# XuanchenLi/Topo4D

Hardware: AMD Instinct MI355X
Metric: rasterizer fwd+bwd views/sec (higher is better)
Workload: dtype f32

## Files before the change

### topo4d_amd/csrc/t4d_raster_gaussian_bwd.h

```cpp
__device__ __forceinline__ void preprocess_bwd(const KP &kp)
{
    const uint32_t nblocks = (uint32_t)(kp.P + kBlock - 1) / kBlock;
    const uint32_t n_pv = gaussian_grid(kp.P, kp.V);
    const bool spare = blockIdx.x >= n_pv;
    uint32_t gb = 0, vb = 0;
    if (!spare && !block_and_view(blockIdx.x, (uint32_t)kp.V, nblocks, gb, vb)) return;
    const int v = spare ? (int)(blockIdx.x - n_pv) : (int)vb;
    const int g = (int)gb * kBlock + threadIdx.x;
    if (spare) {
        __shared__ float s_w[4];
        const float4 *td = reinterpret_cast<const float4 *>(kp.tile_dot) + (size_t)v * kp.T;
        const float *vb = kp.views + (size_t)v * T4D_VIEW_FLOATS + 35;
        const bool black = vb[0] == 0.f && vb[1] == 0.f && vb[2] == 0.f;
        const uint32_t *tc = kp.tile_count + (size_t)v * kp.T;
        float a = 0.f;
        for (int t = threadIdx.x; t < kp.T; t += kBlock) {
            if (tc[t] == 0u && black) continue;
            const float4 d4 = td[t];
            a += (d4.x + d4.y) + (d4.z + d4.w);
        }
        a = wave_sum_to_lane63(a);
        if ((threadIdx.x & 63) == 63) s_w[threadIdx.x >> 6] = a;
        __syncthreads();
        if (threadIdx.x == 0) kp.cotangent_dot[v] = kp.status->overflow != 0u ? 0.f : (s_w[0] + s_w[1]) + (s_w[2] + s_w[3]);
        return;
    }
    if (g >= kp.P) return;
    const size_t vg = (size_t)v * kp.P + g;
    const size_t gp = param_row0(kp, v) + (size_t)g;
    const ViewRecord vrec = load_view_record(kp.views, v);
    const float *view = vrec.view, *proj = vrec.proj;
    const uint32_t flag = kp.status->overflow;
    const int radius_in = kp.radii[vg];
    const float2 p2 = kp.xy[vg];
    const uint32_t base = kp.pair_off[vg];
    const float4 cq = kp.conic_opacity[vg];
    const float mean[3] = { kp.means3D[3 * gp], kp.means3D[3 * gp + 1], kp.means3D[3 * gp + 2] };
    float cov3_in[6] = { 0.f, 0.f, 0.f, 0.f, 0.f, 0.f };
    float4 q = make_float4(1.f, 0.f, 0.f, 0.f);
    float sc[3] = { 0.f, 0.f, 0.f };
    if (kp.cov3D_precomp) {
#pragma unroll
        for (int k = 0; k < 6; k++) cov3_in[k] = kp.cov3D_precomp[6 * gp + k];
    } else {
        sc[0] = kp.scales[3 * gp]; sc[1] = kp.scales[3 * gp + 1]; sc[2] = kp.scales[3 * gp + 2];
        q = reinterpret_cast<const float4 *>(kp.rotations)[gp];
    }
    const float4 q_raw = q;
    if (kp.raw_params && !kp.cov3D_precomp) {
        sc[0] = t4d_act_exp(sc[0]); sc[1] = t4d_act_exp(sc[1]); sc[2] = t4d_act_exp(sc[2]);
        q = t4d_act_normalize(q);
    }
    const bool truncated = flag != 0u;
    const int radius = truncated ? 0 : radius_in;

    float gm[3] = { 0.f, 0.f, 0.f }, g2x = 0.f, g2y = 0.f, gop = 0.f;
    float grgb[3] = { 0.f, 0.f, 0.f }, gsc[3] = { 0.f, 0.f, 0.f }, gq[4] = { 0.f, 0.f, 0.f, 0.f };
    float gcov[6] = { 0.f, 0.f, 0.f, 0.f, 0.f, 0.f };

    if (radius > 0) {
        int x0, y0, x1, y1;
        tile_rect(p2.x, p2.y, radius, kp.gx, kp.gy, x0, y0, x1, y1);
        const uint32_t npairs = (uint32_t)((x1 - x0) * (y1 - y0));
        const float2 *gp = reinterpret_cast<const float2 *>(kp.grad_pair) + (size_t)v * kp.cap * (kGP / 2);
        float S0 = 0.f, S1 = 0.f, S2 = 0.f, S3 = 0.f, S4 = 0.f, S5 = 0.f, gdep = 0.f;
        for (uint32_t k = 0; k < npairs; k++) {
            const uint32_t pr = base + k;
            if (pr >= kp.cap) break;
            const float2 *rec = gp + (size_t)pr * (kGP / 2);
            const float2 a0 = rec[0], a1 = rec[1], a2 = rec[2], a3 = rec[3], a4 = rec[4];
            S0 += a0.x; S1 += a0.y; S2 += a1.x; S3 += a1.y;
            S4 += a2.x; S5 += a2.y; grgb[0] += a3.x; grgb[1] += a3.y;
            grgb[2] += a4.x; gdep += a4.y;
        }
        gop = S0;
        g2x = -cq.w * (cq.x * S1 + cq.y * S2) * (0.5f * kp.W);
        g2y = -cq.w * (cq.z * S2 + cq.y * S1) * (0.5f * kp.H);
        const float X = -0.5f * cq.w * S3, Y = -cq.w * S4, Z = -0.5f * cq.w * S5;

        float cov3[6];
        if (kp.cov3D_precomp) {
#pragma unroll
            for (int k = 0; k < 6; k++) cov3[k] = cov3_in[k];
        } else {
            cov3d_from_scale_rot(sc, kp.scale_modifier, q, cov3);
        }
        const float tanx = vrec.tanx, tany = vrec.tany;
        const float fx = kp.W / (2.0f * tanx), fy = kp.H / (2.0f * tany);
        float T0[3], T1[3], t[3];
        bool inx, iny;
        ewa_rows(mean, view, fx, fy, tanx, tany, T0, T1, t, inx, iny);
        float v0[3], v1[3];
        sym3_mul(cov3, T0, v0);
        sym3_mul(cov3, T1, v1);
        const float a = T0[0] * v0[0] + T0[1] * v0[1] + T0[2] * v0[2] + T4D_COV2D_DILATION;
        const float b = T0[0] * v1[0] + T0[1] * v1[1] + T0[2] * v1[2];
        const float c = T1[0] * v1[0] + T1[1] * v1[1] + T1[2] * v1[2] + T4D_COV2D_DILATION;
        const float denom = a * c - b * b;
        const float d2inv = 1.f / ((denom * denom) + T4D_CONIC_BWD_EPS);
        float dL_da = 0.f, dL_db = 0.f, dL_dc = 0.f;
        if (d2inv != 0.f) {
            dL_da = d2inv * (-c * c * X + b * c * Y + (denom - a * c) * Z);
            dL_dc = d2inv * (-a * a * Z + a * b * Y + (denom - a * c) * X);
            dL_db = d2inv * (2.f * b * c * X - (denom + 2.f * b * b) * Y + 2.f * a * b * Z);
            gcov[0] = T0[0] * T0[0] * dL_da + T0[0] * T1[0] * dL_db + T1[0] * T1[0] * dL_dc;
            gcov[3] = T0[1] * T0[1] * dL_da + T0[1] * T1[1] * dL_db + T1[1] * T1[1] * dL_dc;
            gcov[5] = T0[2] * T0[2] * dL_da + T0[2] * T1[2] * dL_db + T1[2] * T1[2] * dL_dc;
            gcov[1] = 2.f * T0[0] * T0[1] * dL_da + (T0[0] * T1[1] + T0[1] * T1[0]) * dL_db + 2.f * T1[0] * T1[1] * dL_dc;
            gcov[2] = 2.f * T0[0] * T0[2] * dL_da + (T0[0] * T1[2] + T0[2] * T1[0]) * dL_db + 2.f * T1[0] * T1[2] * dL_dc;
            gcov[4] = 2.f * T0[2] * T0[1] * dL_da + (T0[1] * T1[2] + T0[2] * T1[1]) * dL_db + 2.f * T1[1] * T1[2] * dL_dc;
        }
        float dJ00 = 0.f, dJ02 = 0.f, dJ11 = 0.f, dJ12 = 0.f;
#pragma unroll
        for (int j = 0; j < 3; j++) {
            const float dT0 = 2.f * v0[j] * dL_da + v1[j] * dL_db;
            const float dT1 = 2.f * v1[j] * dL_dc + v0[j] * dL_db;
            dJ00 += view[j * 4 + 0] * dT0; dJ02 += view[j * 4 + 2] * dT0;
            dJ11 += view[j * 4 + 1] * dT1; dJ12 += view[j * 4 + 2] * dT1;
        }
        const float tz = 1.f / t[2], tz2 = tz * tz, tz3 = tz2 * tz;
        const float dtx = (inx ? 1.f : 0.f) * -fx * tz2 * dJ02;
        const float dty = (iny ? 1.f : 0.f) * -fy * tz2 * dJ12;
        const float dtz = -fx * tz2 * dJ00 - fy * tz2 * dJ11 + (2.f * fx * t[0]) * tz3 * dJ02 + (2.f * fy * t[1]) * tz3 * dJ12;
        gm[0] = view[0] * dtx + view[1] * dty + view[2] * dtz;
        gm[1] = view[4] * dtx + view[5] * dty + view[6] * dtz;
        gm[2] = view[8] * dtx + view[9] * dty + view[10] * dtz;

        const float hx = proj[0] * mean[0] + proj[4] * mean[1] + proj[8] * mean[2] + proj[12];
        const float hy = proj[1] * mean[0] + proj[5] * mean[1] + proj[9] * mean[2] + proj[13];
        const float hw = proj[3] * mean[0] + proj[7] * mean[1] + proj[11] * mean[2] + proj[15];
        const float mw = 1.0f / (hw + T4D_HOM_W_EPS);
        const float mul1 = hx * mw * mw, mul2 = hy * mw * mw;
        gm[0] += (proj[0] * mw - proj[3] * mul1) * g2x + (proj[1] * mw - proj[3] * mul2) * g2y;
        gm[1] += (proj[4] * mw - proj[7] * mul1) * g2x + (proj[5] * mw - proj[7] * mul2) * g2y;
        gm[2] += (proj[8] * mw - proj[11] * mul1) * g2x + (proj[9] * mw - proj[11] * mul2) * g2y;
        gm[0] += view[2] * gdep; gm[1] += view[6] * gdep; gm[2] += view[10] * gdep;

        if (!kp.cov3D_precomp) {
            float R[9];
            quat_rot(q, R);
            const float s[3] = { kp.scale_modifier * sc[0], kp.scale_modifier * sc[1], kp.scale_modifier * sc[2] };
            const float Gs[9] = { gcov[0], 0.5f * gcov[1], 0.5f * gcov[2], 0.5f * gcov[1], gcov[3], 0.5f * gcov[4],
                                  0.5f * gcov[2], 0.5f * gcov[4], gcov[5] };
            float Mp[9], D[9];
#pragma unroll
            for (int r = 0; r < 3; r++)
#pragma unroll
                for (int k = 0; k < 3; k++) Mp[r * 3 + k] = R[r * 3 + k] * s[k];
#pragma unroll
            for (int k = 0; k < 3; k++) {
                float dM[3];
#pragma unroll
                for (int r = 0; r < 3; r++)
                    dM[r] = 2.f * (Gs[r * 3] * Mp[k] + Gs[r * 3 + 1] * Mp[3 + k] + Gs[r * 3 + 2] * Mp[6 + k]);
                gsc[k] = kp.scale_modifier * (dM[0] * R[k] + dM[1] * R[3 + k] + dM[2] * R[6 + k]);
#pragma unroll
                for (int r = 0; r < 3; r++) D[r * 3 + k] = dM[r] * s[k];
            }
            const float r = q.x, x = q.y, y = q.z, z = q.w;
            gq[0] = 2.f * z * (D[3] - D[1]) + 2.f * y * (D[2] - D[6]) + 2.f * x * (D[7] - D[5]);
            gq[1] = 2.f * y * (D[1] + D[3]) + 2.f * z * (D[2] + D[6]) + 2.f * r * (D[7] - D[5]) - 4.f * x * (D[4] + D[8]);
            gq[2] = 2.f * x * (D[1] + D[3]) + 2.f * r * (D[2] - D[6]) + 2.f * z * (D[5] + D[7]) - 4.f * y * (D[0] + D[8]);
            gq[3] = 2.f * r * (D[3] - D[1]) + 2.f * x * (D[2] + D[6]) + 2.f * y * (D[5] + D[7]) - 4.f * z * (D[0] + D[4]);
        }
    }

    if (kp.raw_params && radius > 0) {
        gop = t4d_act_sigmoid_bwd(cq.w, gop);
        if (!kp.cov3D_precomp) {
#pragma unroll
            for (int k = 0; k < 3; k++) gsc[k] = t4d_act_exp_bwd(sc[k], gsc[k]);
            const float4 gr = t4d_act_normalize_bwd(q_raw, make_float4(gq[0], gq[1], gq[2], gq[3]));
            gq[0] = gr.x; gq[1] = gr.y; gq[2] = gr.z; gq[3] = gr.w;
        }
    }
    kp.dL_dmeans3D[vg * 3] = gm[0]; kp.dL_dmeans3D[vg * 3 + 1] = gm[1]; kp.dL_dmeans3D[vg * 3 + 2] = gm[2];
    kp.dL_dmeans2D[vg * 3] = g2x; kp.dL_dmeans2D[vg * 3 + 1] = g2y; kp.dL_dmeans2D[vg * 3 + 2] = 0.f;
    kp.dL_dopacities[vg] = gop;
    if (kp.dL_dcolors) { kp.dL_dcolors[vg * 3] = grgb[0]; kp.dL_dcolors[vg * 3 + 1] = grgb[1]; kp.dL_dcolors[vg * 3 + 2] = grgb[2]; }
    if (kp.cov3D_precomp) {
#pragma unroll
        for (int k = 0; k < 6; k++) kp.dL_dcov3D[vg * 6 + k] = gcov[k];
    } else {
        kp.dL_dscales[vg * 3] = gsc[0]; kp.dL_dscales[vg * 3 + 1] = gsc[1]; kp.dL_dscales[vg * 3 + 2] = gsc[2];
        reinterpret_cast<float4 *>(kp.dL_drotations)[vg] = make_float4(gq[0], gq[1], gq[2], gq[3]);
    }
}

#ifndef T4D_PBWD_WAVES
#define T4D_PBWD_WAVES 7
#endif
__global__ __launch_bounds__(kBlock) __attribute__((amdgpu_waves_per_eu(T4D_PBWD_WAVES, T4D_PBWD_WAVES))) void k_preprocess_bwd(const KP kp)
{
    preprocess_bwd(kp);
}

__global__ __launch_bounds__(kBlock) void k_sh_bwd(const KP kp)
{
    __shared__ float s_bas[kBlock][17];
    __shared__ float s_gc[kBlock][4];
    const int tid = threadIdx.x;
    const uint32_t nblocks = (uint32_t)(kp.P + kBlock - 1) / kBlock;
    uint32_t pblock, vb;
    if (!block_and_view(blockIdx.x, (uint32_t)kp.V, nblocks, pblock, vb)) return;
    const int v = (int)vb;
    const int g0 = (int)pblock * kBlock;
    const int n = min(kBlock, kp.P - g0);
    const int M3 = kp.M * 3;
    if (tid < n) {
        const int g = g0 + tid;
        const size_t vg = (size_t)v * kp.P + g;
        const size_t gp = param_row0(kp, v) + (size_t)g;
        const bool vis = kp.status->overflow == 0u && kp.radii[vg] > 0;
        float gc[3] = { 0.f, 0.f, 0.f };
        float bas[16];
#pragma unroll
        for (int i = 0; i < 16; i++) bas[i] = 0.f;
        if (vis) {
            const float *vr = kp.views + (size_t)v * T4D_VIEW_FLOATS;
            const float d0[3] = { kp.means3D[3 * gp] - vr[32], kp.means3D[3 * gp + 1] - vr[33], kp.means3D[3 * gp + 2] - vr[34] };
            const float len = sqrtf(d0[0] * d0[0] + d0[1] * d0[1] + d0[2] * d0[2]);
            const float d[3] = { d0[0] / len, d0[1] / len, d0[2] / len };
            float bx[16], by[16], bz[16];
            sh_basis(kp.deg, d, bas);
            sh_basis_grad(kp.deg, d, bx, by, bz);
            const uint32_t cl = kp.clamped[vg];
            const float *grgb = kp.dL_dcolors + vg * 3;
            gc[0] = (cl & 1u) ? 0.f : grgb[0]; gc[1] = (cl & 2u) ? 0.f : grgb[1]; gc[2] = (cl & 4u) ? 0.f : grgb[2];
            const int K = (kp.deg + 1) * (kp.deg + 1);
            float gd[3] = { 0.f, 0.f, 0.f };
            const float *sh = kp.shs + gp * M3;
            if ((kp.M & 3) == 0 && K == 16) {
                const float4 *sh4 = reinterpret_cast<const float4 *>(sh);
                float c[48];
#pragma unroll
                for (int i = 0; i < 12; i++) { const float4 t4 = sh4[i]; c[4 * i] = t4.x; c[4 * i + 1] = t4.y; c[4 * i + 2] = t4.z; c[4 * i + 3] = t4.w; }
#pragma unroll
                for (int k = 0; k < 16; k++) {
                    const float t = c[3 * k] * gc[0] + c[3 * k + 1] * gc[1] + c[3 * k + 2] * gc[2];
                    gd[0] += bx[k] * t; gd[1] += by[k] * t; gd[2] += bz[k] * t;
                }
            } else {
#pragma unroll
                for (int k = 0; k < 16; k++) {
                    if (k < K) {
                        const float t = sh[k * 3] * gc[0] + sh[k * 3 + 1] * gc[1] + sh[k * 3 + 2] * gc[2];
                        gd[0] += bx[k] * t; gd[1] += by[k] * t; gd[2] += bz[k] * t;
                    } else {
                        bas[k] = 0.f;
                    }
                }
            }
            const float dot = d[0] * gd[0] + d[1] * gd[1] + d[2] * gd[2];
            float *gm = kp.dL_dmeans3D + vg * 3;
#pragma unroll
            for (int jj = 0; jj < 3; jj++) gm[jj] += (gd[jj] - d[jj] * dot) / len;
        }
#pragma unroll
        for (int i = 0; i < 16; i++) s_bas[tid][i] = bas[i];
        s_gc[tid][0] = gc[0]; s_gc[tid][1] = gc[1]; s_gc[tid][2] = gc[2];
    }
    __syncthreads();
    float *out = kp.dL_dshs + ((size_t)v * kp.P + g0) * M3;
    if (kp.M == 16) {
        float4 *out4 = reinterpret_cast<float4 *>(out);
        for (int i = tid; i < n * 12; i += kBlock) {
            const int slot = i / 12, e0 = (i % 12) * 4;
            float o[4];
#pragma unroll
            for (int e = 0; e < 4; e++) o[e] = s_bas[slot][(e0 + e) / 3] * s_gc[slot][(e0 + e) % 3];
            out4[i] = make_float4(o[0], o[1], o[2], o[3]);
        }
    } else {
        for (int i = tid; i < n * M3; i += kBlock) {
            const int slot = i / M3, e = i % M3, k = e / 3;
            out[i] = k < 16 ? s_bas[slot][k] * s_gc[slot][e % 3] : 0.f;
        }
    }
}

#ifndef T4D_SHB_VIEWS
#define T4D_SHB_VIEWS 8
#endif
__global__ __launch_bounds__(kBlock) void k_sh_bwd16(const KP kp)
{
    constexpr int kPitch = 52;
    __shared__ __attribute__((aligned(16))) float s_raw[kBlock * kPitch];
    float (*s_bas)[17] = reinterpret_cast<float (*)[17]>(s_raw);
    float (*s_gc)[4] = reinterpret_cast<float (*)[4]>(s_raw + kBlock * 17);
    static_assert(kBlock * 17 + kBlock * 4 <= kBlock * kPitch && (kBlock * 17) % 4 == 0, "the exchange arrays live inside the staging area");
    const int tid = threadIdx.x;
    const uint32_t nblocks = (uint32_t)(kp.P + kBlock - 1) / kBlock;
    const uint32_t ngroups = (uint32_t)(kp.V + T4D_SHB_VIEWS - 1) / T4D_SHB_VIEWS;
    uint32_t pblock, vgrp;
    if (!block_and_view(blockIdx.x, ngroups, nblocks, pblock, vgrp)) return;
    const int g0 = (int)pblock * kBlock;
    const int n = min(kBlock, kp.P - g0);
    const size_t row0 = param_row0(kp, (int)vgrp * T4D_SHB_VIEWS);
    {
        const float4 *src = reinterpret_cast<const float4 *>(kp.shs + (row0 + (size_t)g0) * 48);
        for (int i = tid; i < n * 12; i += kBlock) {
            const int r = i / 12, part = i - r * 12;
            *reinterpret_cast<float4 *>(s_raw + r * kPitch + part * 4) = src[i];
        }
    }
    __syncthreads();
    float c[48];
#pragma unroll
    for (int i = 0; i < 12; i++) {
        const float4 t4 = *reinterpret_cast<const float4 *>(s_raw + min(tid, n - 1) * kPitch + 4 * i);
        c[4 * i] = t4.x; c[4 * i + 1] = t4.y; c[4 * i + 2] = t4.z; c[4 * i + 3] = t4.w;
    }
    __syncthreads();
    const int g = g0 + min(tid, n - 1);
    const float mean[3] = { kp.means3D[3 * (row0 + (size_t)g)], kp.means3D[3 * (row0 + (size_t)g) + 1], kp.means3D[3 * (row0 + (size_t)g) + 2] };
    const bool truncated = kp.status->overflow != 0u;
    const int v_end = min(kp.V, (int)(vgrp + 1u) * T4D_SHB_VIEWS);
    for (int v = (int)vgrp * T4D_SHB_VIEWS; v < v_end; v++) {
        if (tid < n) {
            const size_t vg = (size_t)v * kp.P + g;
            const bool vis = !truncated && kp.radii[vg] > 0;
            float gc[3] = { 0.f, 0.f, 0.f };
            float bas[16];
#pragma unroll
            for (int i = 0; i < 16; i++) bas[i] = 0.f;
            if (vis) {
                const float *vr = kp.views + (size_t)v * T4D_VIEW_FLOATS;
                const float d0[3] = { mean[0] - vr[32], mean[1] - vr[33], mean[2] - vr[34] };
                const float len = sqrtf(d0[0] * d0[0] + d0[1] * d0[1] + d0[2] * d0[2]);
                const float d[3] = { d0[0] / len, d0[1] / len, d0[2] / len };
                float bx[16], by[16], bz[16];
                sh_basis(3, d, bas);
                sh_basis_grad(3, d, bx, by, bz);
                const uint32_t cl = kp.clamped[vg];
                const float *grgb = kp.dL_dcolors + vg * 3;
                gc[0] = (cl & 1u) ? 0.f : grgb[0]; gc[1] = (cl & 2u) ? 0.f : grgb[1]; gc[2] = (cl & 4u) ? 0.f : grgb[2];
                float gd[3] = { 0.f, 0.f, 0.f };
#pragma unroll
                for (int k = 0; k < 16; k++) {
                    const float t = c[3 * k] * gc[0] + c[3 * k + 1] * gc[1] + c[3 * k + 2] * gc[2];
                    gd[0] += bx[k] * t; gd[1] += by[k] * t; gd[2] += bz[k] * t;
                }
                const float dot = d[0] * gd[0] + d[1] * gd[1] + d[2] * gd[2];
                float *gm = kp.dL_dmeans3D + vg * 3;
#pragma unroll
                for (int jj = 0; jj < 3; jj++) gm[jj] += (gd[jj] - d[jj] * dot) / len;
            }
#pragma unroll
            for (int i = 0; i < 16; i++) s_bas[tid][i] = bas[i];
            s_gc[tid][0] = gc[0]; s_gc[tid][1] = gc[1]; s_gc[tid][2] = gc[2];
        }
        __syncthreads();
        float4 *out4 = reinterpret_cast<float4 *>(kp.dL_dshs + ((size_t)v * kp.P + g0) * 48);
        for (int i = tid; i < n * 12; i += kBlock) {
            const int slot = i / 12, e0 = (i - slot * 12) * 4;
            float o[4];
#pragma unroll
            for (int e = 0; e < 4; e++) o[e] = s_bas[slot][(e0 + e) / 3] * s_gc[slot][(e0 + e) % 3];
            out4[i] = make_float4(o[0], o[1], o[2], o[3]);
        }
        __syncthreads();
    }
}

constexpr int kDotBlocks = 64;

__global__ __launch_bounds__(kBlock) void k_view_dot_partial(const float *a, const float *b, size_t n, float *partial)
{
    __shared__ float s_w[4];
    const int v = blockIdx.y, blk = blockIdx.x, tid = threadIdx.x;
    const float *pa = a + (size_t)v * n, *pb = b + (size_t)v * n;
    const size_t per = (((n + kDotBlocks - 1) / kDotBlocks) + 3) & ~(size_t)3;
    const size_t lo = min(n, (size_t)blk * per), hi = min(n, lo + per);
    float acc = 0.f;
    if ((n & 3) == 0 && (((uintptr_t)a | (uintptr_t)b) & 15) == 0) {
        for (size_t i = lo + (size_t)tid * 4; i < hi; i += (size_t)kBlock * 4) {
            const float4 x = *reinterpret_cast<const float4 *>(pa + i), y = *reinterpret_cast<const float4 *>(pb + i);
            acc += (x.x * y.x + x.y * y.y) + (x.z * y.z + x.w * y.w);
        }
    } else {
        for (size_t k = lo + tid; k < hi; k += kBlock) acc += pa[k] * pb[k];
    }
    acc = wave_sum_to_lane63(acc);
    if ((tid & 63) == 63) s_w[tid >> 6] = acc;
    __syncthreads();
    if (tid == 0) partial[(size_t)v * kDotBlocks + blk] = (s_w[0] + s_w[1]) + (s_w[2] + s_w[3]);
}

__global__ __launch_bounds__(64) void k_view_dot_final(const float *partial, float *out)
{
    const int v = blockIdx.x;
    float x = partial[(size_t)v * kDotBlocks + threadIdx.x];
    x = wave_sum_to_lane63(x);
    if (threadIdx.x == 63) out[v] = x;
}

__global__ __launch_bounds__(kBlock) void k_mark_visible(int P, const float *means3D, const float *view, uint8_t *present)
{
#pragma clang fp contract(off)
    const int g = blockIdx.x * kBlock + threadIdx.x;
    if (g >= P) return;
    const float z = view[2] * means3D[3 * (size_t)g] + view[6] * means3D[3 * (size_t)g + 1] +
                    view[10] * means3D[3 * (size_t)g + 2] + view[14];
    present[g] = z > T4D_NEAR_CULL_Z ? 1 : 0;
}
```

### topo4d_amd/csrc/t4d_raster_render_bwd.h

```cpp
__device__ __forceinline__ void tile_pixel_bwd(int tid, int tx, int ty, int &px, int &py)
{
    const int w = tid >> 6, r = (tid >> 4) & 3, i = tid & 15;
    px = tx * T4D_TILE_X + ((w & 1) << 3) + ((r & 1) << 2) + (i >> 2);
    py = ty * T4D_TILE_Y + ((w >> 1) << 3) + ((r >> 1) << 2) + (i & 3);
}

__device__ __forceinline__ int fwd_thread_of(int tid) { return (tid & ~15) | ((tid & 3) << 2) | ((tid >> 2) & 3); }

struct RowWeights { float X, ks, kg; };

__device__ __forceinline__ RowWeights row_weights(const int lane)
{
    const int r = lane >> 4, i = lane & 15, bank = i >> 2, b1 = (i >> 1) & 1;
    RowWeights k;
    k.X = (float)(((r & 1) << 2) + (i >> 2)) - 3.5f;
    const float y0 = (float)((r >> 1) << 2) - 3.5f;
    const float Y = y0 + (float)(i & 3), Yp = y0 + (float)((i & 3) ^ 2);
    auto Ka = [&](float y) { return bank == 1 ? y * y : (bank == 3 ? 0.f : 1.f); };
    auto Kb = [&](float y) { return (bank & 1) ? 0.f : y; };
    k.ks = b1 ? Kb(Y) : Ka(Y);
    k.kg = b1 ? Kb(Yp) : Ka(Yp);
    return k;
}

template <bool NINE>
__device__ __forceinline__ float reduce_moments_row(const float e, const float ex, const float exx, const float c0, const float c1,
                                                    const float c2, const float cd, const RowWeights &k)
{
    float a, b, c;
#define T4D_RED_X                                                                                     \
        "s_nop 1\n\t"                                                                                 \
        "v_add_f32_dpp %[a], %[v0], %[v0] row_ror:8 row_mask:0xf bank_mask:0xf\n\t"                   \
        "v_add_f32_dpp %[b], %[v2], %[v2] row_ror:8 row_mask:0xf bank_mask:0xf\n\t"                   \
        "v_add_f32_dpp %[c], %[v4], %[v4] row_ror:8 row_mask:0xf bank_mask:0xf\n\t"                   \
        "v_add_f32_dpp %[a], %[v1], %[v1] row_ror:8 row_mask:0xf bank_mask:0xc\n\t"                   \
        "v_add_f32_dpp %[b], %[v3], %[v3] row_ror:8 row_mask:0xf bank_mask:0xc\n\t"                   \
        "v_add_f32_dpp %[c], %[v5], %[v5] row_ror:8 row_mask:0xf bank_mask:0xc\n\t"
#define T4D_RED_X4                                                                                    \
        "v_add_f32_dpp %[a], %[a], %[a] row_shl:4 row_mask:0xf bank_mask:0x5\n\t"                     \
        "v_add_f32_dpp %[a], %[b], %[b] row_shr:4 row_mask:0xf bank_mask:0xa\n\t"                     \
        "v_add_f32_dpp %[b], %[c], %[c] row_shl:4 row_mask:0xf bank_mask:0x5\n\t"                     \
        "v_add_f32_dpp %[b], %[c], %[c] row_shr:4 row_mask:0xf bank_mask:0xa\n\t"
#define T4D_RED_OUT [a] "=&v"(a), [b] "=&v"(b), [c] "=&v"(c)
#define T4D_RED_IN [v0] "v"(exx), [v1] "v"(c0), [v2] "v"(c1), [v3] "v"(c2), [v4] "v"(e), [v5] "v"(ex), [ks] "v"(k.ks), [kg] "v"(k.kg), \
                   [m0] "s"(0xaaaaaaaaaaaaaaaaull)
    if (NINE) {
        asm(T4D_RED_X T4D_RED_X4
            "v_add_f32_dpp %[a], %[a], %[a] quad_perm:[2,3,0,1] row_mask:0xf bank_mask:0xf\n\t"
            "v_mul_f32_e32 %[c], %[b], %[ks]\n\t"
            "v_fmac_f32_dpp %[c], %[b], %[kg] quad_perm:[2,3,0,1] row_mask:0xf bank_mask:0xf\n\t"
            "v_cndmask_b32_e64 %[b], %[a], %[c], %[m0]\n\t"
            "v_cndmask_b32_e64 %[c], %[c], %[a], %[m0]\n\t"
            "s_nop 0\n\t"
            "v_add_f32_dpp %[c], %[b], %[c] quad_perm:[1,0,3,2] row_mask:0xf bank_mask:0xf"
            : T4D_RED_OUT : T4D_RED_IN);
        return c;
    } else {
        float d;
        asm(T4D_RED_X
            "v_add_f32_dpp %[d], %[v6], %[v6] row_ror:8 row_mask:0xf bank_mask:0xf\n\t"
            T4D_RED_X4
            "v_add_f32_dpp %[d], %[d], %[d] row_ror:4 row_mask:0xf bank_mask:0xf\n\t"
            "v_cndmask_b32_e64 %[c], %[d], %[a], %[m1]\n\t"
            "v_cndmask_b32_e64 %[d], %[a], %[d], %[m1]\n\t"
            "v_mul_f32_e32 %[a], %[b], %[ks]\n\t"
            "v_fmac_f32_dpp %[a], %[b], %[kg] quad_perm:[2,3,0,1] row_mask:0xf bank_mask:0xf\n\t"
            "v_add_f32_dpp %[d], %[c], %[d] quad_perm:[2,3,0,1] row_mask:0xf bank_mask:0xf\n\t"
            "v_cndmask_b32_e64 %[b], %[d], %[a], %[m0]\n\t"
            "v_cndmask_b32_e64 %[a], %[a], %[d], %[m0]\n\t"
            "s_nop 0\n\t"
            "v_add_f32_dpp %[a], %[b], %[a] quad_perm:[1,0,3,2] row_mask:0xf bank_mask:0xf"
            : T4D_RED_OUT, [d] "=&v"(d) : T4D_RED_IN, [v6] "v"(cd), [m1] "s"(0xccccccccccccccccull));
        return a;
    }
#undef T4D_RED_X
#undef T4D_RED_X4
#undef T4D_RED_OUT
#undef T4D_RED_IN
}

__device__ __forceinline__ int row10_index(const int lane)
{
    const int b0 = lane & 1, b1 = (lane >> 1) & 1, bank = (lane >> 2) & 3;
    if (!b0) {
        if (bank == 0) return b1 ? 2 : 0;
        if (bank == 1) return b1 ? -1 : 5;
        if (bank == 2) return b1 ? 4 : 1;
        return -1;
    }
    if (!b1) return bank == 0 ? 3 : (bank == 1 ? 7 : (bank == 2 ? 6 : 8));
    return bank == 0 ? 9 : -1;
}

__device__ __forceinline__ void moments_about_centre(float (&m)[10], const float pxf, const float pyf)
{
    const double px = pxf, py = pyf, M00 = m[0], M10 = m[1], M01 = m[2], M20 = m[3], M11 = m[4], M02 = m[5];
    const double sx = fma(px, M00, -M10), sy = fma(py, M00, -M01);
    m[1] = (float)sx; m[2] = (float)sy;
    m[3] = (float)fma(px, sx, -fma(px, M10, -M20));
    m[4] = (float)fma(px, sy, -fma(py, M10, -M11));
    m[5] = (float)fma(py, sy, -fma(py, M01, -M02));
}

__device__ __forceinline__ float moment_e(const float e) { return __uint_as_float(__float_as_uint(e) & 0xffffffc0u); }

__device__ __forceinline__ uint32_t row_max_u32(uint32_t v)
{
    v = max(v, (uint32_t)__builtin_amdgcn_update_dpp(0, (int)v, 0xB1, 0xf, 0xf, true));
    v = max(v, (uint32_t)__builtin_amdgcn_update_dpp(0, (int)v, 0x4E, 0xf, 0xf, true));
    v = max(v, (uint32_t)__builtin_amdgcn_update_dpp(0, (int)v, 0x141, 0xf, 0xf, true));
    v = max(v, (uint32_t)__builtin_amdgcn_update_dpp(0, (int)v, 0x140, 0xf, 0xf, true));
    return v;
}

#ifndef T4D_BWD_WAVES
#define T4D_BWD_WAVES 5
#endif
#ifndef T4D_SEG_WAVES
#define T4D_SEG_WAVES 5
#endif
#ifndef T4D_BWD_DA_WAVES
#define T4D_BWD_DA_WAVES T4D_BWD_WAVES
#endif
#define T4D_BWD_NW (LAT ? 2 : (SEGN != 0 ? T4D_SEG_WAVES : (DA ? T4D_BWD_DA_WAVES : T4D_BWD_WAVES)))
#define T4D_BWD_ATTR __attribute__((amdgpu_waves_per_eu(LAT ? 1 : T4D_BWD_NW, T4D_BWD_NW)))
constexpr int kAcc = 10;
constexpr int kEmptySpan = 64;
template <bool DA, bool LAT, int SEGN, bool LONG = false>
__global__ __launch_bounds__(kBlock) T4D_BWD_ATTR void k_render_bwd(const KP kp)
{
    constexpr bool SEG = SEGN != 0;
    constexpr int kSeg = SEG ? SEGN : ::kSeg;
    constexpr int kBwdBatch = SEG ? SEGN : ::kBwdBatch;
    constexpr int kSlabs = LAT ? 16 : 4;
    constexpr int kChunks = (kBwdBatch + 63) / 64;
    constexpr int kListStride = kBwdBatch + 4;
    constexpr int kEnt = 40;
    static_assert(kBwdBatch % 64 == 0, "staged slots come in chunks of one per lane");
    static_assert(kGP == kAcc, "the slab entry and the scratch record hold the same ten sums");
    static_assert(kAcc * 4 == kEnt, "a slab entry and a staged record must have the same stride");
    struct __attribute__((aligned(16))) Shared {
        unsigned char rec[(kBwdBatch + 1) * kEnt];
        float acc[kSlabs][kBwdBatch + 1][kAcc];
        unsigned short list[4][4][kListStride];
        float cut_r2[kChunks * 64];
        uint32_t pair[kBwdBatch];
        uint32_t wmax[4];
    };
    static_assert(((kBwdBatch + 1) * kEnt) % 8 == 0 && (sizeof(float) * kSlabs * (kBwdBatch + 1) * kAcc) % 8 == 0 &&
                  (sizeof(unsigned short) * 16 * kListStride) % 8 == 0, "8-byte members must stay 8-byte aligned");
    __shared__ Shared sh;
    auto &s_rec = sh.rec;
    auto &s_pair = sh.pair;
    auto &s_acc = sh.acc;
    auto &s_r2 = sh.cut_r2;
    auto &s_wmax = sh.wmax;
    auto &s_list = sh.list;
    constexpr int kNull = kBwdBatch;

    const int tid = threadIdx.x;
    const int wave = __builtin_amdgcn_readfirstlane(tid >> 6), lane = tid & 63, row = lane >> 4;
    const int my_slot = (!DA && row10_index(lane & 15) == 9) ? -1 : row10_index(lane & 15);
    const RowWeights rw = row_weights(lane);
    if (tid == 0) {
#pragma unroll
        for (int k = 0; k < kEnt / 8; k++) reinterpret_cast<float2 *>(s_rec + kNull * kEnt)[k] = make_float2(0.f, 0.f);
    }
    if (blockIdx.x >= kp.tile_blocks) {
        const uint32_t spans = (uint32_t)(kp.T + kEmptySpan - 1) / kEmptySpan;
        const uint32_t j = blockIdx.x - kp.tile_blocks;
        const int v = (int)(j / spans), t0 = (int)(j % spans) * kEmptySpan;
        const float *vb = kp.views + (size_t)v * T4D_VIEW_FLOATS + 35;
        const float b0 = vb[0], b1 = vb[1], b2 = vb[2];
        if (b0 == 0.f && b1 == 0.f && b2 == 0.f) return;
        const size_t HWe = (size_t)kp.H * kp.W;
        const float *dc = kp.dL_dcolor + (size_t)v * 3 * HWe;
        for (int t = t0; t < min(t0 + kEmptySpan, kp.T); t++) {
            if (kp.tile_count[(size_t)v * kp.T + t] != 0u) continue;
            const int ty = t / kp.gx, tx = t - ty * kp.gx;
            int ex, ey;
            tile_pixel(tid, tx, ty, ex, ey);
            float d = 0.f;
            if (ex < kp.W && ey < kp.H) {
                const size_t pe = (size_t)ey * kp.W + ex;
                d = fmaf(b0, dc[pe], fmaf(b1, dc[HWe + pe], b2 * dc[2 * HWe + pe]));
            }
            d = wave_sum_to_lane63(d);
            if (lane == 63) kp.tile_dot[((size_t)v * kp.T + t) * 4 + wave] = d;
        }
        return;
    }
    uint4 it;
    if (SEG && !LONG) {
        it = kp.slot_tab[blockIdx.x];
        if (it.w == 0u) return;
    }
    for (int i = tid; i < kSlabs * (kBwdBatch + 1) * kAcc; i += kBlock) (&s_acc[0][0][0])[i] = 0.f;
    for (uint32_t item = blockIdx.x; item < (SEG ? (LONG ? kp.status->live_segments : blockIdx.x + 1u) : (uint32_t)(kp.V * kp.T)); item += kp.tile_blocks) {
    if (SEG && LONG) it = kp.slot_tab[kp.live[item]];
    if (!SEG) it = kp.items[item];
    const int seg_j = SEG ? (int)(it.w & 0x7fffffffu) : 0;
    const int v = (int)(it.x >> 20), t_ = (int)(it.x & 0xfffffu);
    const int ty = t_ / kp.gx, tx = t_ - ty * kp.gx;
    const uint32_t off = it.y, n = it.z;
    if (n == 0) break;
    if (!SEG && LONG && n >= kp.seg_min_pairs &&
        kp.slot_tab[(size_t)v * kp.slots_per_view + seg_slot0(kp, off, (uint32_t)t_)].w != 0u) continue;
    const unsigned long long *keys = kp.keys + (size_t)v * kp.cap + off;
    const float *r2_in = kp.cut_r2 + (size_t)v * kp.cap + off;
    const float2 *xy = kp.xy + (size_t)v * kp.P;
    const float4 *co = kp.conic_opacity + (size_t)v * kp.P;
    const float *rgb = kp.shs ? kp.rgb + (size_t)v * kp.P * 3 : kp.colors_precomp + 3 * param_row0(kp, v);
    const int32_t *radii = kp.radii + (size_t)v * kp.P;
    const uint32_t *pair_off = kp.pair_off + (size_t)v * kp.P;
    float2 *grad_pair = reinterpret_cast<float2 *>(kp.grad_pair) + (size_t)v * kp.cap * (kGP / 2);
    const float *vr = kp.views + (size_t)v * T4D_VIEW_FLOATS;

    int px, py;
    tile_pixel_bwd(tid, tx, ty, px, py);
    const bool inside = px < kp.W && py < kp.H;
    const v2f pix_f = { (float)px, (float)py };
    const size_t HW = (size_t)kp.H * kp.W, pix = (size_t)py * kp.W + px;

    float T_final = 0.f, dp0 = 0.f, dp1 = 0.f, dp2 = 0.f, ddep = 0.f, dalp = 0.f;
    uint32_t last_contributor = 0;
    if (inside) {
        T_final = kp.final_T[(size_t)v * HW + pix];
        last_contributor = kp.n_contrib[(size_t)v * HW + pix];
        const float *dc = kp.dL_dcolor + (size_t)v * 3 * HW;
        dp0 = dc[pix]; dp1 = dc[HW + pix]; dp2 = dc[2 * HW + pix];
        if (DA && kp.dL_ddepth) ddep = kp.dL_ddepth[(size_t)v * HW + pix];
        if (DA && kp.dL_dalpha) dalp = kp.dL_dalpha[(size_t)v * HW + pix];
    }
    const v2f dp01 = { dp0, dp1 };
    float T = T_final;
    float acc = vr[35] * dp0 + vr[36] * dp1 + vr[37] * dp2;
    const int nb = (int)((n + kBwdBatch - 1) / kBwdBatch);
    if (SEG && seg_j + 1 < nb) {
        const uint32_t p = (uint32_t)(seg_j + 1) * kSeg;
        if (last_contributor > p) {
            const float *sb = kp.snap + ((size_t)v * kp.slots_per_view + seg_slot0(kp, off, (uint32_t)t_)) * (kSnapFloats * kBlock) + fwd_thread_of(tid);
            const float *sp = sb + (size_t)seg_j * (kSnapFloats * kBlock), *sf = sb + (size_t)(nb - 1) * (kSnapFloats * kBlock);
            const float Tp = sp[0];
            float suf = fmaf(sf[kBlock] - sp[kBlock], dp0, fmaf(sf[2 * kBlock] - sp[2 * kBlock], dp1, (sf[3 * kBlock] - sp[3 * kBlock]) * dp2));
            if (DA) suf = fmaf(sf[4 * kBlock] - sp[4 * kBlock], ddep, suf) + (Tp - T_final) * dalp;
            acc = fmaf(T_final, acc, suf) / Tp;
            T = Tp;
        }
    }

    const uint32_t rmax_v = row_max_u32(last_contributor);
    uint32_t row_max[4];
#pragma unroll
    for (int r = 0; r < 4; r++) row_max[r] = lane_value(rmax_v, 16 * r);
    const uint32_t wave_max = max(max(row_max[0], row_max[1]), max(row_max[2], row_max[3]));
    if (lane == 0) s_wmax[wave] = wave_max;
    __syncthreads();
    const uint32_t tile_max = max(max(s_wmax[0], s_wmax[1]), max(s_wmax[2], s_wmax[3]));

    for (int bi = SEG ? seg_j : nb - 1; bi >= (SEG ? seg_j : 0); bi--) {
        const uint32_t lo = (uint32_t)bi * kBwdBatch;
        const int cnt = (int)min((uint32_t)kBwdBatch, n - lo);
        const bool live = lo < tile_max;
        if (tid < cnt) s_pair[tid] = 0xffffffffu;
        if (tid < kChunks * 64) {
            float r2 = -1.f;
            float2 p = make_float2(0.f, 0.f);
            if (tid < cnt) {
                const unsigned long long key = keys[lo + tid];
                const float r2_kept = live ? r2_in[lo + tid] : -1.f;
                const uint32_t g = (uint32_t)key;
                if (g < (uint32_t)kp.P) {
                    const float2 pg = xy[g];
                    const int rad = radii[g];
                    const uint32_t po = pair_off[g];
                    float4 c = make_float4(0.f, 0.f, 0.f, 0.f);
                    float c0 = 0.f, c1 = 0.f, c2 = 0.f;
                    if (live) { c = co[g]; c0 = rgb[3 * (size_t)g]; c1 = rgb[3 * (size_t)g + 1]; c2 = rgb[3 * (size_t)g + 2]; }
                    p = pg;
                    int x0, y0, x1, y1;
                    tile_rect(pg.x, pg.y, rad, kp.gx, kp.gy, x0, y0, x1, y1);
                    const int local = (ty - y0) * (x1 - x0) + (tx - x0);
                    s_pair[tid] = (tx >= x0 && tx < x1 && ty >= y0 && ty < y1) ? po + (uint32_t)local : 0xffffffffu;
                    if (live) {
                        const float4 q4 = scale_conic(c);
                        float2 *rec = reinterpret_cast<float2 *>(s_rec + tid * kEnt);
                        rec[0] = make_float2(q4.x, q4.y); rec[1] = make_float2(q4.z, q4.w);
                        rec[2] = make_float2(c0, c1);
                        rec[3] = make_float2(c2, __uint_as_float((uint32_t)(key >> 32)));
                        r2 = r2_kept;
                    }
                }
            }
            if (live) {
                reinterpret_cast<float2 *>(s_rec + tid * kEnt)[4] = p;
                s_r2[tid] = r2;
            }
        }
        __syncthreads();
        if (live) {
            unsigned long long mt[4][kChunks];
#pragma unroll
            for (int c2 = 0; c2 < kChunks; c2++) {
                const int slot = (c2 << 6) + lane;
                unsigned long long mc[4] = { 0ull, 0ull, 0ull, 0ull };
                if ((c2 << 6) < cnt)
                    wave_touch_masks(reinterpret_cast<const float2 *>(s_rec + slot * kEnt)[4], s_r2[slot], tx, ty, wave, mc);
#pragma unroll
                for (int r = 0; r < 4; r++) mt[r][c2] = mc[r];
            }
            int nsteps = 0, cnts[4];
#pragma unroll
            for (int r = 0; r < 4; r++) {
                unsigned long long m[kChunks];
#pragma unroll
                for (int c2 = 0; c2 < kChunks; c2++) {
                    m[c2] = mt[r][c2];
                    const uint32_t base = lo + ((uint32_t)c2 << 6);
                    if (row_max[r] <= base) m[c2] = 0;
                    else if (row_max[r] - base < 64u) m[c2] &= (1ull << (row_max[r] - base)) - 1ull;
                }
                cnts[r] = build_visit_list<kChunks, true, kEnt>(m, s_list[wave][r], lane);
                nsteps = max(nsteps, cnts[r]);
            }
#pragma unroll
            for (int r = 0; r < 4; r++) pad_visit_list(s_list[wave][r], cnts[r], nsteps, lane, (unsigned short)(kNull * kEnt));
            __builtin_amdgcn_wave_barrier();
            unsigned long long conflict[kChunks];
#pragma unroll
            for (int c2 = 0; c2 < kChunks; c2++) {
                conflict[c2] = 0ull;
                if (!LAT && (c2 << 6) < nsteps) {
                    const int st = (c2 << 6) + lane;
                    const unsigned short *l0 = s_list[wave][0];
                    const uint32_t e0 = l0[st], e1 = l0[kListStride + st], e2 = l0[2 * kListStride + st], e3 = l0[3 * kListStride + st];
                    const uint32_t nul = (uint32_t)(kNull * kEnt);
                    const bool same = st < nsteps && ((e0 == e1 && e0 != nul) || (e0 == e2 && e0 != nul) || (e0 == e3 && e0 != nul) ||
                                                      (e1 == e2 && e1 != nul) || (e1 == e3 && e1 != nul) || (e2 == e3 && e2 != nul));
                    conflict[c2] = __ballot(same);
                }
            }
            unsigned long long conflict_s[kChunks];
#pragma unroll
            for (int c2 = 0; c2 < kChunks; c2++) conflict_s[c2] = uniform_u64(conflict[c2]);
            const unsigned short *list = s_list[wave][row];
            const unsigned char *rec_b = s_rec;
            unsigned char *slab = LAT ? reinterpret_cast<unsigned char *>(my_slot >= 0 ? &s_acc[wave * 4 + row][0][my_slot]
                                                                                      : &s_acc[wave * 4 + row][kNull][(lane & 15) % kAcc])
                                      : reinterpret_cast<unsigned char *>(&s_acc[wave][0][0] + (my_slot >= 0 ? my_slot : 0));
            const uint32_t slab_and = (!LAT || my_slot >= 0) ? 0xffffffffu : 0u;
            const int lc_rel = (int)min(last_contributor - min(last_contributor, lo), (uint32_t)kBwdBatch) * kEnt;
            uint2 pk = *reinterpret_cast<const uint2 *>(list);
            for (int k = 0; k < nsteps; k += 4) {
                const uint32_t ee[4] = { pk.x & 0xffffu, pk.x >> 16, pk.y & 0xffffu, pk.y >> 16 };
                pk = *reinterpret_cast<const uint2 *>(list + k + 4);
                float Gs[4], alphas[4];
                float4 cds[4];
                bool contribs[4];
#pragma unroll
                for (int u = 0; u < 4; u++) {
                    const float2 *rec = reinterpret_cast<const float2 *>(rec_b + ee[u]);
                    const float2 q01 = rec[0], q23 = rec[1], c01 = rec[2], c23 = rec[3];
                    const v2f d = *reinterpret_cast<const v2f *>(rec + 4) - pix_f;
                    cds[u] = make_float4(c01.x, c01.y, c23.x, c23.y);
                    float p2;
                    eval_splat(make_float4(q01.x, q01.y, q23.x, q23.y), d, p2, Gs[u], alphas[u]);
                    contribs[u] = (int)ee[u] < lc_rel && !(p2 > 0.0f) && !(alphas[u] < T4D_ALPHA_MIN);
                }
                const uint32_t cbits = (uint32_t)(conflict_s[kChunks == 1 ? 0 : (k >> 6)] >> (k & 63));
#pragma unroll
                for (int u = 0; u < 4; u++) {
                    const bool contrib = contribs[u];
                    const float G = Gs[u], alpha = alphas[u];
                    float *dst = reinterpret_cast<float *>(slab + (LAT ? (ee[u] & slab_and) : ee[u]));
                    const float old = *dst;
                    float e = 0.f, w = 0.f;
                    if (LAT) {
                        const float4 cd = cds[u];
                        const float om = 1.f - alpha;
                        const float inv = __builtin_amdgcn_rcpf(om);
                        const float Tn = T * inv;
                        float q = fmaf(cd.x, dp01.x, fmaf(cd.y, dp01.y, cd.z * dp2));
                        if (DA) q = fmaf(cd.w, ddep, q) + dalp;
                        const float qma = q - acc;
                        const float dL_dalpha = qma * Tn;
                        T = contrib ? Tn : T;
                        w = contrib ? alpha * Tn : 0.f;
                        e = contrib ? G * dL_dalpha : 0.f;
                        acc = contrib ? fmaf(alpha, qma, acc) : acc;
                    } else if (contrib) {
                        const float4 cd = cds[u];
                        const float om = 1.f - alpha;
                        const float inv = __builtin_amdgcn_rcpf(om);
                        T = T * inv;
                        w = alpha * T;
                        float q = fmaf(cd.x, dp01.x, fmaf(cd.y, dp01.y, cd.z * dp2));
                        if (DA) q = fmaf(cd.w, ddep, q) + dalp;
                        const float qma = q - acc;
                        const float dL_dalpha = qma * T;
                        e = G * dL_dalpha;
                        acc = fmaf(alpha, qma, acc);
                    }
                    e = moment_e(e);
                    const float ex = e * rw.X;
                    const v2f wdp = w * dp01;
                    const float tot = reduce_moments_row<!DA>(e, ex, ex * rw.X, wdp.x, wdp.y, w * dp2, DA ? w * ddep : 0.f, rw);
                    const bool add = my_slot >= 0;
                    if (LAT) {
                        *dst = old + tot;
                    } else if (!((cbits >> u) & 1u)) {
                        if (add) *dst = old + tot;
                    } else {
#pragma unroll
                        for (int rr = 0; rr < 4; rr++) {
                            if (add && row == rr) *dst += tot;
                            __builtin_amdgcn_fence(__ATOMIC_RELEASE, "wavefront");
                            __builtin_amdgcn_wave_barrier();
                        }
                    }
                }
            }
        }
        __syncthreads();
        if (tid < cnt) {
            float a[10];
#pragma unroll
            for (int k = 0; k < 10; k++) a[k] = 0.f;
            const float2 pc = live ? reinterpret_cast<const float2 *>(s_rec + tid * kEnt)[4] : make_float2(0.f, 0.f);
#pragma unroll 1
            for (int w = 0; w < 4; w++) {
                float m[10];
#pragma unroll
                for (int k = 0; k < 10; k++) m[k] = 0.f;
#pragma unroll
                for (int s = 0; s < kSlabs / 4; s++) {
                    float2 *src = reinterpret_cast<float2 *>(&s_acc[w * (kSlabs / 4) + s][tid][0]);
#pragma unroll
                    for (int k = 0; k < 5; k++) {
                        const float2 b2 = src[k];
                        m[2 * k] += b2.x; m[2 * k + 1] += b2.y;
                        src[k] = make_float2(0.f, 0.f);
                    }
                }
                moments_about_centre(m, pc.x - ((float)(tx * T4D_TILE_X + ((w & 1) << 3)) + 3.5f),
                                        pc.y - ((float)(ty * T4D_TILE_Y + ((w >> 1) << 3)) + 3.5f));
#pragma unroll
                for (int k = 0; k < 10; k++) a[k] += m[k];
            }
            const uint32_t pr = s_pair[tid];
            if (pr < kp.cap) {
#pragma unroll
                for (int k = 0; k < kGP / 2; k++) grad_pair[(size_t)pr * (kGP / 2) + k] = make_float2(a[2 * k], a[2 * k + 1]);
            }
        }
        __syncthreads();
    }
    if (kp.tile_dot && seg_j == 0) {
        const float d = wave_sum_to_lane63(acc);
        if (lane == 63) kp.tile_dot[((size_t)v * kp.T + t_) * 4 + wave] = d;
    }
    }
}
```

Measured before the change: 56360.

## Stage per-pair gradient records in LDS and defer non-LAT slab accumulation

In preprocess_bwd, each block now computes the min/max range of pair records its threads own and cooperatively streams that range through a shared-memory staging buffer in chunks with unrolled coalesced loads. This replaces per-thread strided global reads of the pair records. Out-of-range threads now stay alive so they can join the barriers. In the render backward kernel, per-block setup is moved after the early-exit checks for empty items. The non-LAT path also gathers its four reduced totals first and does the read-modify-write slab updates afterwards. The costs are extra LDS use (checked by a static_assert against seven workgroups per CU), block-wide syncs per chunk, and idle threads when pair ranges are sparse.

```diff
diff --git a/topo4d_amd/csrc/t4d_raster_gaussian_bwd.h b/topo4d_amd/csrc/t4d_raster_gaussian_bwd.h
--- a/topo4d_amd/csrc/t4d_raster_gaussian_bwd.h
+++ b/topo4d_amd/csrc/t4d_raster_gaussian_bwd.h
@@ -1,3 +1,10 @@
+#ifndef T4D_PAIR_CHUNK
+#define T4D_PAIR_CHUNK 512
+#endif
+constexpr int kPairChunk = T4D_PAIR_CHUNK;
+constexpr int kPairLoads = 5;
+static_assert(7 * (kPairChunk * kGP * 4 + 64) <= 160 * 1024, "the staging chunk must leave k_preprocess_bwd its seven workgroups per CU");
+
 __device__ __forceinline__ void preprocess_bwd(const KP &kp)
 {
     const uint32_t nblocks = (uint32_t)(kp.P + kBlock - 1) / kBlock;
@@ -25,9 +32,9 @@
         if (threadIdx.x == 0) kp.cotangent_dot[v] = kp.status->overflow != 0u ? 0.f : (s_w[0] + s_w[1]) + (s_w[2] + s_w[3]);
         return;
     }
-    if (g >= kp.P) return;
-    const size_t vg = (size_t)v * kp.P + g;
-    const size_t gp = param_row0(kp, v) + (size_t)g;
+    const bool in_range = g < kp.P;
+    const size_t vg = (size_t)v * kp.P + min(g, kp.P - 1);
+    const size_t gp = param_row0(kp, v) + (size_t)min(g, kp.P - 1);
     const ViewRecord vrec = load_view_record(kp.views, v);
     const float *view = vrec.view, *proj = vrec.proj;
     const uint32_t flag = kp.status->overflow;
@@ -52,27 +59,59 @@
         q = t4d_act_normalize(q);
     }
     const bool truncated = flag != 0u;
-    const int radius = truncated ? 0 : radius_in;
+    const int radius = (truncated || !in_range) ? 0 : radius_in;
 
     float gm[3] = { 0.f, 0.f, 0.f }, g2x = 0.f, g2y = 0.f, gop = 0.f;
     float grgb[3] = { 0.f, 0.f, 0.f }, gsc[3] = { 0.f, 0.f, 0.f }, gq[4] = { 0.f, 0.f, 0.f, 0.f };
     float gcov[6] = { 0.f, 0.f, 0.f, 0.f, 0.f, 0.f };
 
-    if (radius > 0) {
+    __shared__ float2 s_stage[kPairChunk * (kGP / 2)];
+    __shared__ uint32_t s_lo[4], s_hi[4];
+    uint32_t my_n = 0;
+    if (radius > 0 && base < kp.cap) {
         int x0, y0, x1, y1;
         tile_rect(p2.x, p2.y, radius, kp.gx, kp.gy, x0, y0, x1, y1);
-        const uint32_t npairs = (uint32_t)((x1 - x0) * (y1 - y0));
-        const float2 *gp = reinterpret_cast<const float2 *>(kp.grad_pair) + (size_t)v * kp.cap * (kGP / 2);
-        float S0 = 0.f, S1 = 0.f, S2 = 0.f, S3 = 0.f, S4 = 0.f, S5 = 0.f, gdep = 0.f;
-        for (uint32_t k = 0; k < npairs; k++) {
-            const uint32_t pr = base + k;
-            if (pr >= kp.cap) break;
-            const float2 *rec = gp + (size_t)pr * (kGP / 2);
-            const float2 a0 = rec[0], a1 = rec[1], a2 = rec[2], a3 = rec[3], a4 = rec[4];
-            S0 += a0.x; S1 += a0.y; S2 += a1.x; S3 += a1.y;
-            S4 += a2.x; S5 += a2.y; grgb[0] += a3.x; grgb[1] += a3.y;
-            grgb[2] += a4.x; gdep += a4.y;
-        }
+        my_n = min((uint32_t)((x1 - x0) * (y1 - y0)), kp.cap - base);
+    }
+    float S0 = 0.f, S1 = 0.f, S2 = 0.f, S3 = 0.f, S4 = 0.f, S5 = 0.f, gdep = 0.f;
+    {
+        uint32_t lo = my_n ? base : 0xffffffffu, hi = my_n ? base + my_n : 0u;
+#pragma unroll
+        for (int d = 32; d > 0; d >>= 1) {
+            lo = min(lo, (uint32_t)__shfl_xor((int)lo, d, 64));
+            hi = max(hi, (uint32_t)__shfl_xor((int)hi, d, 64));
+        }
+        if ((threadIdx.x & 63) == 0) { s_lo[threadIdx.x >> 6] = lo; s_hi[threadIdx.x >> 6] = hi; }
+        __syncthreads();
+        lo = min(min(s_lo[0], s_lo[1]), min(s_lo[2], s_lo[3]));
+        hi = max(max(s_hi[0], s_hi[1]), max(s_hi[2], s_hi[3]));
+        const float2 *recs = reinterpret_cast<const float2 *>(kp.grad_pair) + (size_t)v * kp.cap * (kGP / 2);
+        uint32_t k = 0;
+        for (uint32_t c0 = lo; c0 < hi; c0 += kPairChunk) {
+            const uint32_t c1 = c0 + min((uint32_t)kPairChunk, hi - c0), words = (c1 - c0) * (kGP / 2);
+            const float2 *src = recs + (size_t)c0 * (kGP / 2);
+            for (uint32_t i0 = threadIdx.x; i0 < words; i0 += kPairLoads * kBlock) {
+                float2 t[kPairLoads];
+#pragma unroll
+                for (int j = 0; j < kPairLoads; j++)
+                    if (i0 + j * kBlock < words) t[j] = src[i0 + j * kBlock];
+#pragma unroll
+                for (int j = 0; j < kPairLoads; j++)
+                    if (i0 + j * kBlock < words) s_stage[i0 + j * kBlock] = t[j];
+            }
+            __syncthreads();
+            const uint32_t end = min(my_n, c1 - min(base, c1));
+            for (; k < end; k++) {
+                const float2 *rec = s_stage + (size_t)(base + k - c0) * (kGP / 2);
+                const float2 a0 = rec[0], a1 = rec[1], a2 = rec[2], a3 = rec[3], a4 = rec[4];
+                S0 += a0.x; S1 += a0.y; S2 += a1.x; S3 += a1.y;
+                S4 += a2.x; S5 += a2.y; grgb[0] += a3.x; grgb[1] += a3.y;
+                grgb[2] += a4.x; gdep += a4.y;
+            }
+            __syncthreads();
+        }
+    }
+    if (radius > 0) {
         gop = S0;
         g2x = -cq.w * (cq.x * S1 + cq.y * S2) * (0.5f * kp.W);
         g2y = -cq.w * (cq.z * S2 + cq.y * S1) * (0.5f * kp.H);
@@ -174,6 +213,7 @@
             gq[0] = gr.x; gq[1] = gr.y; gq[2] = gr.z; gq[3] = gr.w;
         }
     }
+    if (!in_range) return;
     kp.dL_dmeans3D[vg * 3] = gm[0]; kp.dL_dmeans3D[vg * 3 + 1] = gm[1]; kp.dL_dmeans3D[vg * 3 + 2] = gm[2];
     kp.dL_dmeans2D[vg * 3] = g2x; kp.dL_dmeans2D[vg * 3 + 1] = g2y; kp.dL_dmeans2D[vg * 3 + 2] = 0.f;
     kp.dL_dopacities[vg] = gop;
diff --git a/topo4d_amd/csrc/t4d_raster_render_bwd.h b/topo4d_amd/csrc/t4d_raster_render_bwd.h
--- a/topo4d_amd/csrc/t4d_raster_render_bwd.h
+++ b/topo4d_amd/csrc/t4d_raster_render_bwd.h
@@ -160,12 +160,6 @@
 
     const int tid = threadIdx.x;
     const int wave = __builtin_amdgcn_readfirstlane(tid >> 6), lane = tid & 63, row = lane >> 4;
-    const int my_slot = (!DA && row10_index(lane & 15) == 9) ? -1 : row10_index(lane & 15);
-    const RowWeights rw = row_weights(lane);
-    if (tid == 0) {
-#pragma unroll
-        for (int k = 0; k < kEnt / 8; k++) reinterpret_cast<float2 *>(s_rec + kNull * kEnt)[k] = make_float2(0.f, 0.f);
-    }
     if (blockIdx.x >= kp.tile_blocks) {
         const uint32_t spans = (uint32_t)(kp.T + kEmptySpan - 1) / kEmptySpan;
         const uint32_t j = blockIdx.x - kp.tile_blocks;
@@ -194,6 +188,16 @@
     if (SEG && !LONG) {
         it = kp.slot_tab[blockIdx.x];
         if (it.w == 0u) return;
+    } else if (SEG) {
+        if (blockIdx.x >= kp.status->live_segments) return;
+    } else {
+        if (blockIdx.x >= (uint32_t)(kp.V * kp.T) || kp.items[blockIdx.x].z == 0u) return;
+    }
+    const int my_slot = (!DA && row10_index(lane & 15) == 9) ? -1 : row10_index(lane & 15);
+    const RowWeights rw = row_weights(lane);
+    if (tid == 0) {
+#pragma unroll
+        for (int k = 0; k < kEnt / 8; k++) reinterpret_cast<float2 *>(s_rec + kNull * kEnt)[k] = make_float2(0.f, 0.f);
     }
     for (int i = tid; i < kSlabs * (kBwdBatch + 1) * kAcc; i += kBlock) (&s_acc[0][0][0])[i] = 0.f;
     for (uint32_t item = blockIdx.x; item < (SEG ? (LONG ? kp.status->live_segments : blockIdx.x + 1u) : (uint32_t)(kp.V * kp.T)); item += kp.tile_blocks) {
@@ -368,12 +372,14 @@
                     contribs[u] = (int)ee[u] < lc_rel && !(p2 > 0.0f) && !(alphas[u] < T4D_ALPHA_MIN);
                 }
                 const uint32_t cbits = (uint32_t)(conflict_s[kChunks == 1 ? 0 : (k >> 6)] >> (k & 63));
+                float tots[4];
 #pragma unroll
                 for (int u = 0; u < 4; u++) {
                     const bool contrib = contribs[u];
                     const float G = Gs[u], alpha = alphas[u];
                     float *dst = reinterpret_cast<float *>(slab + (LAT ? (ee[u] & slab_and) : ee[u]));
-                    const float old = *dst;
+                    float old = 0.f;
+                    if (LAT) old = *dst;
                     float e = 0.f, w = 0.f;
                     if (LAT) {
                         const float4 cd = cds[u];
@@ -405,17 +411,23 @@
                     const float ex = e * rw.X;
                     const v2f wdp = w * dp01;
                     const float tot = reduce_moments_row<!DA>(e, ex, ex * rw.X, wdp.x, wdp.y, w * dp2, DA ? w * ddep : 0.f, rw);
+                    if (LAT) *dst = old + tot;
+                    else tots[u] = tot;
+                }
+                if (!LAT) {
                     const bool add = my_slot >= 0;
-                    if (LAT) {
-                        *dst = old + tot;
-                    } else if (!((cbits >> u) & 1u)) {
-                        if (add) *dst = old + tot;
-                    } else {
-#pragma unroll
-                        for (int rr = 0; rr < 4; rr++) {
-                            if (add && row == rr) *dst += tot;
-                            __builtin_amdgcn_fence(__ATOMIC_RELEASE, "wavefront");
-                            __builtin_amdgcn_wave_barrier();
+#pragma unroll
+                    for (int u = 0; u < 4; u++) {
+                        float *dst = reinterpret_cast<float *>(slab + ee[u]);
+                        if (!((cbits >> u) & 1u)) {
+                            if (add) *dst += tots[u];
+                        } else {
+#pragma unroll
+                            for (int rr = 0; rr < 4; rr++) {
+                                if (add && row == rr) *dst += tots[u];
+                                __builtin_amdgcn_fence(__ATOMIC_RELEASE, "wavefront");
+                                __builtin_amdgcn_wave_barrier();
+                            }
                         }
                     }
                 }
```

Result: no change. 56320 (-0.1%).
